# skmhrk1209/VSRD

Hardware: AMD Instinct MI355X
Metric: rendered rays/sec (fwd+bwd) per GPU, KITTI-360 376×1408, 16 instances (higher is better)
Workload: dtype f32

## Files before the change

__graft_entry__.py:

```python
import os
import subprocess
import sys

ROOT = os.path.dirname(os.path.abspath(__file__))
if ROOT not in sys.path:
    sys.path.insert(0, ROOT)

CSRC = os.path.join(ROOT, "vsrd_amd", "csrc")
LIB_DIR = os.path.join(ROOT, "vsrd_amd", "lib")
LIB = os.path.join(LIB_DIR, "libvsrd_hip.so")
HIPCC = os.environ.get("HIPCC", "/opt/rocm/bin/hipcc")
COMMON_FLAGS = ["--offload-arch=gfx950", "-O3", "-std=c++17", "-fPIC", "-ffp-contract=fast"]
if os.environ.get("VSRD_SLP", "0") != "1":
    COMMON_FLAGS.append("-fno-slp-vectorize")
COMMON_FLAGS += os.environ.get("VSRD_HIPCC_EXTRA", "").split()
SCHED_FLAGS = [] if os.environ.get("VSRD_SCHED", "iterative-ilp") == "default" else \
    ["-mllvm", "-amdgpu-sched-strategy=" + os.environ.get("VSRD_SCHED", "iterative-ilp")]
UNITS = [("api.hip", SCHED_FLAGS), ("split_front.hip", [])]
HIPCC_FLAGS = COMMON_FLAGS + SCHED_FLAGS


def _stale(target, sources):
    if not os.path.exists(target):
        return True
    t = os.path.getmtime(target)
    return any(os.path.getmtime(s) > t for s in sources)


def compile_library(output, extra_flags=()):
    staged = f"{output}.{os.getpid()}.tmp.so"
    objects, running = [], []
    try:
        for name, unit_flags in UNITS:
            obj = f"{output}.{os.getpid()}.{name}.o"
            objects.append(obj)
            running.append(subprocess.Popen([HIPCC, *COMMON_FLAGS, *unit_flags, *extra_flags, "-c", os.path.join(CSRC, name), "-o", obj], cwd=ROOT))
        codes = [p.wait() for p in running]
        if any(codes):
            raise subprocess.CalledProcessError(next(c for c in codes if c), "hipcc -c")
        subprocess.run([HIPCC, "--offload-arch=gfx950", "-shared", "-fPIC", "-o", staged, *objects], check=True, cwd=ROOT)
        os.replace(staged, output)
    finally:
        for path in [staged, *objects]:
            if os.path.exists(path):
                os.remove(path)


def build(force=False):
    os.makedirs(LIB_DIR, exist_ok=True)
    sources = [os.path.join(CSRC, f) for f in sorted(os.listdir(CSRC))]
    sources.append(os.path.join(ROOT, "include", "vsrd_hip.h"))
# ... 64 lines not shown
```

include/vsrd_hip.h:

```cpp
#ifndef VSRD_HIP_H
#define VSRD_HIP_H

#include <stddef.h>
#include <stdint.h>

#ifdef __cplusplus
extern "C" {
#endif

#define VSRD_ABI_VERSION 12

#define VSRD_OK 0
#define VSRD_E_INVALID_ARGUMENT (-1)
#define VSRD_E_UNSUPPORTED (-2)
#define VSRD_E_LAUNCH (-3)
#define VSRD_E_WORKSPACE (-4)

#define VSRD_MAX_INSTANCES 64
#define VSRD_MAX_SAMPLES 256
#define VSRD_INSTANCE_STRIDE 16
#define VSRD_MLP_WEIGHTS 1617

#define VSRD_FRAME_HEADER_HAS_VIEWS 0x10000
typedef struct vsrd_frame_header {
// ... 310 lines not shown
} vsrd_frame_log_config;

int32_t vsrd_frame_log(const vsrd_frame_log_config* log, void* stream);

#define VSRD_PATCH_MAX_VIEWS 32
#define VSRD_PATCH_MAX_PIXELS 256
#define VSRD_PATCH_MAX_RAYS 65535
typedef struct vsrd_patch_correlation_config {
    int32_t num_views;
    int32_t num_rays;
    int32_t height, width;
    int32_t patch_width;
    int32_t patch_height;
    int32_t top_k;
    int32_t target_view;
    float sample_epsilon;
    float correlation_epsilon;
} vsrd_patch_correlation_config;

int32_t vsrd_grayscale_images(const float* images, int32_t num_views, int32_t height, int32_t width, float* gray, void* stream);

size_t vsrd_patch_correlation_workspace_bytes(int32_t num_views, int32_t num_rays, int32_t patch_pixels);

int32_t vsrd_patch_correlation_forward(const vsrd_patch_correlation_config* config, const float* gray, const float* intrinsics, const float* extrinsics,
                                       const int32_t* pixels, const float* positions, const float* normals, const uint8_t* converged,
                                       void* workspace, size_t workspace_bytes, float* loss, float* stats,
                                       float* patches, float* coefficients, int32_t* selected, void* stream);

int32_t vsrd_patch_correlation_backward(const vsrd_patch_correlation_config* config, const float* gray, const float* intrinsics, const float* extrinsics,
                                        const int32_t* pixels, const float* positions, const float* normals, const uint8_t* converged,
                                        void* workspace, size_t workspace_bytes, const float* stats, const float* grad_loss,
                                        float* grad_positions, float* grad_normals, void* stream);

#define VSRD_HYPER_LAYERS 5
#define VSRD_HYPER_WIDTH 256
typedef struct vsrd_hypernetwork {
    int32_t num_instances;
    int32_t num_outputs;
    float beta1, beta2, adam_epsilon, lr_gamma;
    vsrd_adam_tensors embeddings;
    vsrd_adam_tensors weight_v[VSRD_HYPER_LAYERS];
    vsrd_adam_tensors weight_g[VSRD_HYPER_LAYERS];
    vsrd_adam_tensors bias[VSRD_HYPER_LAYERS];
    vsrd_adam_tensors norm_weight[VSRD_HYPER_LAYERS - 1];
    vsrd_adam_tensors norm_bias[VSRD_HYPER_LAYERS - 1];
    int32_t num_frames;
    int64_t frame_stride;
} vsrd_hypernetwork;

size_t vsrd_hypernetwork_workspace_bytes(int32_t num_instances);

int32_t vsrd_hypernetwork_forward(const vsrd_hypernetwork* net, void* workspace, size_t workspace_bytes,
                                  float* mlp_weights, float* centred, void* stream);

int32_t vsrd_hypernetwork_backward_step(const vsrd_hypernetwork* net, void* workspace, size_t workspace_bytes,
                                        const float* grad_mlp_weights, float grad_scale, void* stream);

int32_t vsrd_hypernetwork_forward_with_header(const vsrd_hypernetwork* net, void* workspace, size_t workspace_bytes,
                                              float* mlp_weights, float* centred, const vsrd_frame_header* frame_header, void* stream);
int32_t vsrd_hypernetwork_backward_step_with_header(const vsrd_hypernetwork* net, void* workspace, size_t workspace_bytes,
                                                    const float* grad_mlp_weights, float grad_scale, const vsrd_frame_header* frame_header, void* stream);

int32_t vsrd_centre_mlp_weights(const float* mlp_weights, int32_t num_instances, float* centred, void* stream);

int32_t vsrd_selftest_wave(const float* in64, float* out576, void* stream);
int32_t vsrd_selftest_gelu(const float* x, int32_t n, float* out, void* stream);
// ... 6 lines not shown
```

vsrd_amd/csrc/api.hip:

```cpp
#include <cstdio>
#include <cstdlib>
#include "../../include/vsrd_hip.h"
#include "aux_kernels.h"
#include "quad_step.h"
#include "matching.h"
#include "ray_sampling.h"
#include "projection.h"
#include "frame_step.h"
#include "hypernetwork.h"
#include "frame_ingest.h"
#include "frame_labels.h"
#include "frame_group_labels.h"
#include "frame_masks.h"
#include "frame_metrics.h"
#include "frame_log.h"
#include "patch_correlation.h"
#include "launch.h"

namespace {

using namespace vsrd;

constexpr int kMaxBlocks = 16384;

// ... 194 lines not shown
    bool rows;
    bool quad, full;
    int lanes, rays_per_wave, shape_instances;
    int rounds;
    size_t lds_floats;
    size_t num_groups;
    size_t flag_bytes;
};
RowsPlan plan_rows(int num_instances, int num_distances, int num_rays, uint32_t flags, bool allowed) {
    RowsPlan r = {};
    r.rows = allowed && !(flags & VSRD_FLAG_STEP_WAVE_PER_RAY) && num_instances <= kPairMaxInstances && num_distances <= 2 * kPairMaxSamples;
    if (!r.rows) return r;
    const int S = (num_distances + 1) / 2;
    r.quad = num_instances <= kQuadMaxInstances && num_distances <= 2 * kQuadMaxSamples;
    r.lanes = r.quad ? kRowLanes : 32;
    r.rays_per_wave = kWave / r.lanes;
    r.shape_instances = r.quad ? kQuadMaxInstances : kPairMaxInstances;
    r.full = num_distances == 8 * r.lanes && 2 * num_instances > r.shape_instances && !switches().no_full_shape;
    r.rounds = (r.quad && S <= r.lanes) ? 1 : (S <= 2 * r.lanes ? 2 : 4);
    r.lds_floats = static_cast<size_t>(quad_lds_floats(S, r.full ? r.shape_instances : num_instances, r.lanes));
    r.num_groups = (static_cast<size_t>(num_rays) + r.rays_per_wave - 1) / r.rays_per_wave;
    r.flag_bytes = 16 + ((r.num_groups + 15) & ~static_cast<size_t>(15));
    return r;
}

bool cap_to_workspace(size_t bytes, int width, size_t flag_bytes, Geometry* g) {
    const int waves_per_block = g->threads / kWave;
    if (flag_bytes + static_cast<size_t>(waves_per_block) * width * sizeof(float) > bytes) return false;
    const int max_waves = static_cast<int>((bytes - flag_bytes) / sizeof(float) / width);
    if (g->blocks * waves_per_block > max_waves) g->blocks = max_waves / waves_per_block;
    return true;
}

template <typename Kernel, typename... Args>
void launch_hot_then_rest(Kernel hot, Kernel rest, const Geometry& g, hipStream_t s, Args... args) {
    hipLaunchKernelGGL(hot, dim3(g.blocks), dim3(g.threads), g.lds_bytes, s, args...);
    hipLaunchKernelGGL(rest, dim3(g.blocks), dim3(g.threads), g.lds_bytes, s, args...);
}

constexpr size_t kSeedBudgetBytes = size_t(6) << 30;
constexpr int kFrontBlocks = 512;
constexpr int kMlpAdjointBlocks = 4096;
constexpr int kPairBlocks = 1024;

struct ResidualStepPlan {
    int rounds, chunk, front_blocks, front_waves, slots_per_item, items_per_instance;
    bool pair;
    long long slots_per_instance;
    size_t front_lds;
    size_t box_partials, loss_partials, jets, box_extra, counter, segment_sums, seeds, item_rows, masks, item_flags, images, total_bytes;
};

long long size_chunk(ResidualStepPlan* p, long long chunk, int N) {
    p->chunk = static_cast<int>(chunk);
    const long long want = (chunk + kMaxWavesPerBlock - 1) / kMaxWavesPerBlock;
    p->front_blocks = static_cast<int>(want > kFrontBlocks ? kFrontBlocks : want);
    p->front_waves = p->front_blocks * kMaxWavesPerBlock;
    p->slots_per_instance = chunk * p->rounds;
    return (p->slots_per_instance * N) / 16384;
}

void lay_out(ResidualStepPlan* p, int N, long long per_item, size_t loss_floats, bool with_images) {
    p->slots_per_item = static_cast<int>(per_item);
    p->items_per_instance = static_cast<int>((p->slots_per_instance + per_item - 1) / per_item);
    size_t at = 0;
    auto take = [&](size_t floats) { const size_t here = at; at += (floats + 3) & ~size_t(3); return here; };
// ... 375 lines not shown
    if (residual && config->num_rays > 0 && !(config->flags & VSRD_FLAG_RESIDUAL_SINGLE_KERNEL)) {
        bool taken = false;
        const int32_t status = render_backward_split(field, config, origins, directions, distances, num_distances, grad_labels, grad_gradients,
                                                     grad_weights, workspace, workspace_bytes, grad_instances, grad_mlp_weights, stream, &taken);
        if (taken) return status;
    }
    const hipStream_t s = static_cast<hipStream_t>(stream);
    const int row = N * kGradStride;
    const int mlp_row = N * kMlpWeights;
    if (config->num_rays == 0) {
        if (residual && hipMemsetAsync(grad_mlp_weights, 0, mlp_row * sizeof(float), s) != hipSuccess) return VSRD_E_LAUNCH;
        return hipMemsetAsync(grad_instances, 0, row * sizeof(float), s) == hipSuccess ? VSRD_OK : VSRD_E_LAUNCH;
    }
    Geometry g;
    const FieldArgs f = field_args(field);
    RenderArgs c = render_args(config);
    c.sh.inv_t = f.inv_t;
    const RowsPlan r = plan_rows(N, num_distances, config->num_rays, config->flags, !residual && !grad_gradients && !grad_weights);
    if (r.rows) {
        if (!plan(static_cast<int>(r.num_groups), r.lds_floats, &g)) return VSRD_E_UNSUPPORTED;
        if (!cap_to_workspace(workspace_bytes, row, r.flag_bytes, &g)) return VSRD_E_WORKSPACE;
        const int num_waves = g.blocks * (g.threads / kWave);
        float* partials = static_cast<float*>(workspace);
        unsigned char* redo_flags = reinterpret_cast<unsigned char*>(partials + static_cast<size_t>(num_waves) * row);
        if (hipMemsetAsync(redo_flags, 0, 16, s) != hipSuccess) return VSRD_E_LAUNCH;
        for_bool(r.full, [&](auto full) {
            auto launch = [&](auto hot, auto rest) {
                launch_hot_then_rest(hot, rest, g, s, f, field->instances, c, origins, directions, distances, num_distances, grad_labels, partials, redo_flags);
            };
            if (r.quad) launch(render_backward_quad_kernel<true, decltype(full)::value>, render_backward_quad_kernel<false, false>);
            else launch(render_backward_pair_kernel<true, decltype(full)::value>, render_backward_pair_kernel<false, false>);
        });
        if (launch_status() != VSRD_OK) return VSRD_E_LAUNCH;
        hipLaunchKernelGGL(reduce_partials_kernel, dim3(row), dim3(256), 0, s, partials, num_waves, row, grad_instances);
        return launch_status();
    }
    if (!plan(config->num_rays, static_cast<size_t>(backward_lds_floats(num_distances, N, residual)), &g)) return VSRD_E_UNSUPPORTED;
    if (residual && g.threads > kResidualWaves * kWave) return VSRD_E_UNSUPPORTED;
    if (residual && g.blocks > kMaxBlocksResidual) g.blocks = kMaxBlocksResidual;
    const OneKernelWorkspace w = one_kernel_workspace(workspace, N, residual);
    bool known = false;
    for_bool(residual, [&](auto res) {
        known = for_rounds<1, 2, 4>(rounds_for(num_distances - 1), [&](auto k) {
            constexpr auto kernel = render_backward_kernel<decltype(k)::value, decltype(res)::value>;
            fit_to_residency(kernel, &g);
            if (residual && g.blocks > kMaxBlocksResidual) g.blocks = kMaxBlocksResidual;
            hipLaunchKernelGGL(kernel, dim3(g.blocks), dim3(g.threads), g.lds_bytes, s, f, field->instances, field->mlp_weights, c, origins, directions, distances,
                               num_distances, grad_labels, grad_gradients, grad_weights, w.partials, w.mlp_partials, w.jets, w.seeds);
        });
    });
    if (!known) return VSRD_E_UNSUPPORTED;
    if (launch_status() != VSRD_OK) return VSRD_E_LAUNCH;
    const int num_waves = g.blocks * (g.threads / kWave);
    hipLaunchKernelGGL(reduce_partials_kernel, dim3(row), dim3(256), 0, s, w.partials, num_waves, row, grad_instances);
    if (residual)
        hipLaunchKernelGGL(reduce_partials_kernel, dim3(mlp_row), dim3(256), 0, s, w.mlp_partials, num_waves, mlp_row, grad_mlp_weights);
    return launch_status();
}

int32_t vsrd_render_hierarchical_forward(const vsrd_field* field, const vsrd_render_config* config,
                                         const float* origins, const float* directions,
                                         const float* u_coarse, const float* u_fine,
                                         float* labels, float* distances, float* gradients, float* weights, float* coarse_weights,
                                         float* u_coarse_out, float* u_fine_out, void* stream) {
    if (config != nullptr && config->num_frames > 1) return VSRD_E_UNSUPPORTED;
    if (!valid_field(field) || !valid_config(config)) return VSRD_E_INVALID_ARGUMENT;
    if (config->num_rays == 0) return VSRD_OK;
// ... 142 lines not shown
    const int num_waves = g.blocks * (g.threads / kWave);
    float* partials = static_cast<float*>(workspace);
    float* loss_partials = partials + static_cast<size_t>(num_waves) * row;
    unsigned char* redo_flags = reinterpret_cast<unsigned char*>(loss_partials + num_waves);
    int32_t status = VSRD_OK;
    bool known = true;
    if (r.rows) {
        auto launch = [&](auto hot, auto rest) {
            if ((status = opt_in_lds(hot, g.lds_bytes)) != VSRD_OK || (status = opt_in_lds(rest, g.lds_bytes)) != VSRD_OK) return;
            if (hipMemsetAsync(redo_flags, 0, 16, s) != hipSuccess) { status = VSRD_E_LAUNCH; return; }
            launch_hot_then_rest(hot, rest, g, s, f, field->instances, c, origins, directions, u_coarse, u_fine, targets, instance_weights, loss_scale, labels, partials,
                                 loss_partials, redo_flags);
        };
        const bool yaw_only = (config->flags & VSRD_FLAG_YAW_GRADIENTS) != 0u;
        if (r.quad && r.full) for_bool(yaw_only, [&](auto y) {
            launch(render_silhouette_quad_kernel<4, true, true, decltype(y)::value>, render_silhouette_quad_kernel<4, false, false>); });
        else if (r.full) for_bool(yaw_only, [&](auto y) {
            launch(render_silhouette_pair_kernel<4, true, true, decltype(y)::value>, render_silhouette_pair_kernel<4, false, false>); });
        else if (r.quad) known = for_rounds<1, 2, 4>(r.rounds, [&](auto k) {
            launch(render_silhouette_quad_kernel<decltype(k)::value, true, false>, render_silhouette_quad_kernel<decltype(k)::value, false, false>); });
        else known = for_rounds<2, 4>(r.rounds, [&](auto k) {
            launch(render_silhouette_pair_kernel<decltype(k)::value, true, false>, render_silhouette_pair_kernel<decltype(k)::value, false, false>); });
    } else {
        known = for_rounds<1, 2, 4>(rounds, [&](auto k) {
            constexpr auto kernel = render_silhouette_kernel<decltype(k)::value>;
            if ((status = opt_in_lds(kernel, g.lds_bytes)) != VSRD_OK) return;
            hipLaunchKernelGGL(kernel, dim3(g.blocks), dim3(g.threads), g.lds_bytes, s, f, field->instances, c, origins, directions, u_coarse, u_fine, targets,
                               instance_weights, loss_scale, labels, partials, loss_partials);
        });
    }
    if (!known) return VSRD_E_UNSUPPORTED;
    if (status != VSRD_OK) return status;
    if (launch_status() != VSRD_OK) return VSRD_E_LAUNCH;
    hipLaunchKernelGGL(reduce_partials_kernel, dim3(row + 1), dim3(256), 0, s, partials, num_waves, row, grad_instances, nullptr, loss_partials, 1, loss);
    return launch_status();
}

static int32_t residual_step_single_kernel(const vsrd_field* field, const vsrd_render_config* config,
                                  const float* origins, const float* directions, const float* u_coarse, const float* u_fine,
                                  const float* targets, const float* instance_weights, float loss_scale, float eikonal_ratio,
                                  void* workspace, size_t workspace_bytes,
                                  float* losses, float* grad_instances, float* grad_mlp_weights, float* labels, void* stream) {
    if (!valid_field(field) || !valid_config(config, true) || !workspace || !losses || !grad_instances || !grad_mlp_weights) return VSRD_E_INVALID_ARGUMENT;
    if (field->mlp_weights == nullptr) return VSRD_E_INVALID_ARGUMENT;
    const int N = field->num_instances;
    if (workspace_bytes < vsrd_workspace_bytes(N, 1)) return VSRD_E_WORKSPACE;
    const hipStream_t s = static_cast<hipStream_t>(stream);
    const int row = N * kGradStride, mlp_row = N * kMlpWeights;
    if (config->num_rays == 0) {
        if (hipMemsetAsync(losses, 0, 2 * sizeof(float), s) != hipSuccess) return VSRD_E_LAUNCH;
        if (hipMemsetAsync(grad_mlp_weights, 0, mlp_row * sizeof(float), s) != hipSuccess) return VSRD_E_LAUNCH;
        return hipMemsetAsync(grad_instances, 0, row * sizeof(float), s) == hipSuccess ? VSRD_OK : VSRD_E_LAUNCH;
    }
    if (!origins || !directions || !targets) return VSRD_E_INVALID_ARGUMENT;
    const int S = config->num_samples;
    const int num_points = 2 * S - 1;
    const int rounds = rounds_for(num_points);
    Geometry g;
    if (!plan(config->num_rays, static_cast<size_t>(residual_step_lds_floats(S, N)), &g)) return VSRD_E_UNSUPPORTED;
    if (g.threads > kResidualWaves * kWave) return VSRD_E_UNSUPPORTED;
    if (g.blocks > kMaxBlocksResidual) g.blocks = kMaxBlocksResidual;
    const FieldArgs f = field_args(field);
    RenderArgs c = render_args(config);
    c.sh.inv_t = f.inv_t;
    const int num_waves = g.blocks * (g.threads / kWave);
    const OneKernelWorkspace w = one_kernel_workspace(workspace, N, true);
    float* loss_partials = w.partials + static_cast<size_t>(num_waves) * row;
// ... 415 lines not shown

size_t vsrd_patch_correlation_workspace_bytes(int32_t num_views, int32_t num_rays, int32_t patch_pixels) {
    return valid_patch_shape(num_views, num_rays, patch_pixels) ? patch_workspace_floats(num_views, num_rays) * sizeof(float) : 0;
}

int32_t vsrd_patch_correlation_forward(const vsrd_patch_correlation_config* config, const float* gray, const float* intrinsics, const float* extrinsics,
                                       const int32_t* pixels, const float* positions, const float* normals, const uint8_t* converged,
                                       void* workspace, size_t workspace_bytes, float* loss, float* stats,
                                       float* patches, float* coefficients, int32_t* selected, void* stream) {
    PatchArgs a;
    const int32_t status = patch_args(config, gray, intrinsics, extrinsics, pixels, positions, normals, converged, workspace, workspace_bytes, &a);
    if (status != VSRD_OK) return status;
    if (!loss || !stats) return VSRD_E_INVALID_ARGUMENT;
    const hipStream_t s = static_cast<hipStream_t>(stream);
    hipLaunchKernelGGL(patch_constants_kernel, dim3(1), dim3(kWave), 0, s, a);
    hipLaunchKernelGGL(patch_correlation_forward_kernel, dim3(a.num_rays), dim3(kPatchThreads), 0, s, a, patches, coefficients, selected);
    hipLaunchKernelGGL(patch_loss_kernel, dim3(1), dim3(kWave), 0, s, a, loss, stats);
    return launch_status();
}

int32_t vsrd_patch_correlation_backward(const vsrd_patch_correlation_config* config, const float* gray, const float* intrinsics, const float* extrinsics,
                                        const int32_t* pixels, const float* positions, const float* normals, const uint8_t* converged,
                                        void* workspace, size_t workspace_bytes, const float* stats, const float* grad_loss,
                                        float* grad_positions, float* grad_normals, void* stream) {
    PatchArgs a;
    const int32_t status = patch_args(config, gray, intrinsics, extrinsics, pixels, positions, normals, converged, workspace, workspace_bytes, &a);
    if (status != VSRD_OK) return status;
    if (!stats || !grad_loss || !grad_positions || !grad_normals) return VSRD_E_INVALID_ARGUMENT;
    const hipStream_t s = static_cast<hipStream_t>(stream);
    hipLaunchKernelGGL(patch_constants_kernel, dim3(1), dim3(kWave), 0, s, a);
    hipLaunchKernelGGL(patch_correlation_backward_kernel, dim3(a.num_rays), dim3(kPatchThreads), 0, s, a, stats, grad_loss, grad_positions, grad_normals);
    return launch_status();
}

namespace {
struct HyperPlan {
    size_t activations;
    size_t inv_norm;
    size_t gz;
    size_t partials;
    size_t norm_partials;
    size_t total;
    int final_blocks;
};
static HyperPlan plan_hypernetwork(int num_instances) {
    const size_t slab = static_cast<size_t>(num_instances) * kHyperWidth;
    HyperPlan p;
    p.final_blocks = (kMlpWeights + kHyperWaves - 1) / kHyperWaves;
    p.activations = 0;
    p.inv_norm = p.activations + (VSRD_HYPER_LAYERS - 1) * slab;
    p.gz = p.inv_norm + (VSRD_HYPER_LAYERS - 1) * kHyperWidth + kMlpWbarFloats;
    p.partials = p.gz + (VSRD_HYPER_LAYERS) * slab;
    p.norm_partials = p.partials + static_cast<size_t>(p.final_blocks) * slab;
    p.total = p.norm_partials + (VSRD_HYPER_LAYERS - 1) * 2 * slab;
    return p;
}
static bool valid_hypernetwork(const vsrd_hypernetwork* net) {
    if (!net || net->num_instances < 1 || net->num_instances > VSRD_MAX_INSTANCES || net->num_outputs != kMlpWeights) return false;
    if (!valid_adam(net->embeddings)) return false;
    for (int l = 0; l < VSRD_HYPER_LAYERS; ++l) {
        if (!valid_adam(net->weight_v[l]) || !valid_adam(net->weight_g[l]) || !valid_adam(net->bias[l])) return false;
        if (l + 1 < VSRD_HYPER_LAYERS && (!valid_adam(net->norm_weight[l]) || !valid_adam(net->norm_bias[l]))) return false;
    }
    return true;
}
}
// ... 197 lines not shown
```

vsrd_amd/csrc/frame_step.h:

```cpp
#pragma once
#include "matching.h"
#include "projection.h"

namespace vsrd {

constexpr int kFrameThreads = 256;
constexpr int kFrameMaxBoxes = 64;
constexpr int kFrameMaxViews = 32;
constexpr int kBoxEdges = 12;

struct FrameStepArgs {
    int num_boxes, num_views;
    float height, width, epsilon;
    float location_lo[3], location_hi[3], dimension_lo[3], dimension_hi[3];
    int num_steps;
    float max_temperature, min_temperature, max_std, min_std;
    float weight_iou, weight_l1, weight_silhouette;
    float beta1, beta2, adam_epsilon, lr_gamma;
    long long frame_stride;
    const FrameHeader* header;
};

__host__ __device__ constexpr size_t frame_scratch_floats(int num_views, int num_boxes) {
    return static_cast<size_t>(num_views) * num_boxes * (4 + 4 + 4 + 24);
}

__device__ __forceinline__ float lerp_torch(float a, float b, float w) {
    const float diff = b - a;
    return (fabsf(w) < 0.5f) ? (a + w * diff) : (b - diff * (1.0f - w));
}
__device__ __forceinline__ float sigmoid_precise(float x) { return 1.0f / (1.0f + expf(-x)); }

struct DecodedBox {
    float sig_l[3], sig_d[3];
    float loc[3], dim[3];
    float norm, c, s;
};

__device__ __forceinline__ DecodedBox decode_box(const FrameStepArgs& a, const float* raw_loc, const float* raw_dim, const float* raw_ori) {
    DecodedBox b;
#pragma unroll
    for (int j = 0; j < 3; ++j) {
        b.sig_l[j] = sigmoid_precise(raw_loc[j]);
        b.sig_d[j] = sigmoid_precise(raw_dim[j]);
        b.loc[j] = lerp_torch(a.location_lo[j], a.location_hi[j], b.sig_l[j]);
        b.dim[j] = lerp_torch(a.dimension_lo[j], a.dimension_hi[j], b.sig_d[j]);
    }
    b.norm = fmaxf(sqrtf(raw_ori[0] * raw_ori[0] + raw_ori[1] * raw_ori[1]), 1.0e-12f);
    b.c = raw_ori[0] / b.norm;
    b.s = raw_ori[1] / b.norm;
    return b;
}

__device__ __forceinline__ void unit_corner(int k, float* u) {
    const int table[8][3] = {{-1, -1, 1}, {1, -1, 1}, {1, -1, -1}, {-1, -1, -1}, {-1, 1, 1}, {1, 1, 1}, {1, 1, -1}, {-1, 1, -1}};
    u[0] = static_cast<float>(table[k][0]); u[1] = static_cast<float>(table[k][1]); u[2] = static_cast<float>(table[k][2]);
}

__device__ __forceinline__ float dmax_first(float a, float b) { return (a > b) ? 1.0f : ((a == b) ? 0.5f : 0.0f); }
__device__ __forceinline__ float dmin_first(float a, float b) { return (a < b) ? 1.0f : ((a == b) ? 0.5f : 0.0f); }

__device__ __forceinline__ float diou_loss(const float* p, const float* g, float* grad) {
    const float x1 = p[0], y1 = p[1], x2 = p[2], y2 = p[3], x1g = g[0], y1g = g[1], x2g = g[2], y2g = g[3];
    const float eps = 1.0e-7f;
    const float ix1 = fmaxf(x1, x1g), iy1 = fmaxf(y1, y1g), ix2 = fminf(x2, x2g), iy2 = fminf(y2, y2g);
    const bool overlap = (iy2 > iy1) && (ix2 > ix1);
    const float iw = ix2 - ix1, ih = iy2 - iy1;
    const float inter = overlap ? iw * ih : 0.0f;
    const float uni = (x2 - x1) * (y2 - y1) + (x2g - x1g) * (y2g - y1g) - inter;
    const float wx = fmaxf(x2, x2g) - fminf(x1, x1g), wy = fmaxf(y2, y2g) - fminf(y1, y1g);
    const float diagonal = wx * wx + wy * wy + eps;
    const float cxd = (x1 + x2) / 2.0f - (x1g + x2g) / 2.0f, cyd = (y1 + y2) / 2.0f - (y1g + y2g) / 2.0f;
    const float centres = cxd * cxd + cyd * cyd;
    const float ue = uni + eps;
    const float dI[4] = {overlap ? -ih * dmax_first(x1, x1g) : 0.0f, overlap ? -iw * dmax_first(y1, y1g) : 0.0f,
                         overlap ? ih * dmin_first(x2, x2g) : 0.0f, overlap ? iw * dmin_first(y2, y2g) : 0.0f};
    const float dA[4] = {-(y2 - y1), -(x2 - x1), (y2 - y1), (x2 - x1)};
    const float dD[4] = {-2.0f * wx * dmin_first(x1, x1g), -2.0f * wy * dmin_first(y1, y1g), 2.0f * wx * dmax_first(x2, x2g), 2.0f * wy * dmax_first(y2, y2g)};
    const float dC[4] = {cxd, cyd, cxd, cyd};
#pragma unroll
    for (int k = 0; k < 4; ++k) {
        const float dU = dA[k] - dI[k];
        grad[k] = -(dI[k] * ue - inter * dU) / (ue * ue) + (dC[k] * diagonal - centres * dD[k]) / (diagonal * diagonal);
    }
    return 1.0f - inter / ue + centres / diagonal;
}

struct FrameBuffers {
    const float* raw_locations;
// ... 429 lines not shown
```

vsrd_amd/csrc/render_kernels.h:

```cpp
#pragma once
#include "render.h"

namespace vsrd {

constexpr int kMaxWavesPerBlock = 4;
constexpr int kBlockThreads = kMaxWavesPerBlock * kWave;

__device__ __forceinline__ int waves_per_block() { return static_cast<int>(blockDim.x) >> 6; }
constexpr int kGradStride = kInstanceStride;
constexpr int kSeedFloats = 7;
constexpr int kMlpBatch = 8;

__host__ __device__ constexpr int forward_weights_floats(bool residual) { return residual ? kMlpWbarFloats : 0; }

__host__ __device__ constexpr int backward_lds_floats(int num_distances, int num_instances, bool residual) {
    return (forward_weights_floats(residual) + (residual ? kMlpLdsFloats + kMlpBatch * 4 * num_instances : 0) + num_distances + num_instances +
            num_instances * kGradStride + cull_coef_floats(num_instances) + 3) & ~3;
}

__host__ __device__ constexpr int forward_lds_floats(int num_distances, int num_instances, bool residual = false) {
    return (forward_weights_floats(residual) + num_distances + num_instances * kWave + cull_coef_floats(num_instances) + 3) & ~3;
}

__host__ __device__ constexpr int hierarchical_lds_floats(int num_samples, int num_instances, bool residual) {
// ... 1556 lines not shown
        float* dst = box_extra + i * kGradStride + (idx - kMlpWbarFloats);
        *dst = (accumulate ? *dst : 0.0f) + total;
    }
}

__global__ __launch_bounds__(256) void reduce_partials_kernel(const float* __restrict__ partials, int num_waves, int row, float* __restrict__ out,
                                                              const float* __restrict__ extra = nullptr,
                                                              const float* __restrict__ partials2 = nullptr, int row2 = 0, float* __restrict__ out2 = nullptr,
                                                              long long frame_stride = 0, const FrameHeader* __restrict__ frame_header = nullptr) {
    if (frame_stride != 0) {
        const long long shift = frame_shift(frame_stride, blockIdx.y);
        VSRD_OF_FRAME(partials, shift); VSRD_OF_FRAME(out, shift); VSRD_OF_FRAME(extra, shift); VSRD_OF_FRAME(partials2, shift); VSRD_OF_FRAME(out2, shift);
        VSRD_OF_FRAME(frame_header, shift);
    }
    __shared__ float scratch[256 / kWave];
    const bool second = static_cast<int>(blockIdx.x) >= row;
    const int idx = second ? static_cast<int>(blockIdx.x) - row : static_cast<int>(blockIdx.x);
    if (frame_header != nullptr && !second && idx >= frame_count(frame_header, row / kGradStride) * kGradStride) return;
    const float* table = second ? partials2 : partials;
    const int pitch = second ? row2 : row;
    float acc = 0.0f;
    for (int w = threadIdx.x; w < num_waves; w += blockDim.x) acc += table[static_cast<size_t>(w) * pitch + idx];
    acc = wave_sum(acc);
    if (lane_id() == 0) scratch[threadIdx.x >> 6] = acc;
    __syncthreads();
    if (threadIdx.x == 0) {
        float total = 0.0f;
        for (int k = 0; k < 256 / kWave; ++k) total += scratch[k];
        if (second) out2[idx] = total;
        else out[idx] = total + (extra ? extra[idx] : 0.0f);
    }
}

}
```

vsrd_amd/fields.py:

```python
import functools
from dataclasses import dataclass
from typing import Optional

import torch

from . import _lib


class UnsupportedFieldError(TypeError):
    pass


@dataclass
class FieldBlock:
    instances: torch.Tensor
    temperature: float
    mlp_weights: Optional[torch.Tensor]
    label_indices: Optional[torch.Tensor]
    hard: bool = False
    yaw_gradients: bool = False
    capture_key: Optional[tuple] = None

    @property
    def num_instances(self):
        return self.instances.shape[0]


def pack_instances(locations, orientations, dimensions):
    n = locations.shape[0]
    return torch.cat([locations.reshape(n, 3), orientations.reshape(n, 9), dimensions.reshape(n, 3),
                      locations.new_zeros(n, 1)], dim=-1).to(torch.float32).contiguous()



class _Field:

    def __call__(self, positions):
        from .rendering import evaluate_field
        return evaluate_field(self, positions)


class BoxSDF(_Field):

    def __init__(self, dimension):
        self.dimension = dimension


class Rotation(_Field):

    def __init__(self, sdf, rotation_matrix):
        self.sdf, self.rotation_matrix = sdf, rotation_matrix


class Translation(_Field):

    def __init__(self, sdf, translation_vector):
        self.sdf, self.translation_vector = sdf, translation_vector


class ResidualField(_Field):

# ... 206 lines not shown
```

vsrd_amd/models.py:

```python
import math

import torch
import torch.nn as nn
import torch.nn.functional as F

_UNIT_CORNERS = [[-1, -1, 1], [1, -1, 1], [1, -1, -1], [-1, -1, -1], [-1, 1, 1], [1, 1, 1], [1, 1, -1], [-1, 1, -1]]


def yaw_matrix(cos, sin):
    zero, one = torch.zeros_like(cos), torch.ones_like(cos)
    rows = [torch.stack([cos, zero, sin], -1), torch.stack([zero, one, zero], -1), torch.stack([-sin, zero, cos], -1)]
    return torch.stack(rows, -2)


_corner_cache = {}


def _unit_corners(like):
    key = (like.device, like.dtype)
    if key not in _corner_cache:
        _corner_cache[key] = torch.tensor(_UNIT_CORNERS, dtype=like.dtype, device=like.device)
    return _corner_cache[key]


class BoxParameters3D(nn.Module):

    def __init__(self, batch_size, num_instances, num_features=256,
                 location_range=((-50.0, 1.55 - 1.75 / 2.0 - 5.0, 0.0), (50.0, 1.55 - 1.75 / 2.0 + 5.0, 100.0)),
                 dimension_range=((0.75, 0.75, 1.5), (1.0, 1.0, 2.5))):
        super().__init__()
        self.locations = nn.Parameter(torch.zeros(batch_size, num_instances, 3))
        self.dimensions = nn.Parameter(torch.zeros(batch_size, num_instances, 3))
        self.orientations = nn.Parameter(torch.tensor([1.0, 0.0]).repeat(batch_size, num_instances, 1))
        self.embeddings = nn.Parameter(torch.rand(num_features).repeat(batch_size, num_instances, 1))
        self.register_buffer("location_range", torch.as_tensor(location_range, dtype=torch.float32))
        self.register_buffer("dimension_range", torch.as_tensor(dimension_range, dtype=torch.float32))

    def decode_location(self, raw):
        return torch.lerp(self.location_range[0], self.location_range[1], torch.sigmoid(raw))

    def decode_dimension(self, raw):
        return torch.lerp(self.dimension_range[0], self.dimension_range[1], torch.sigmoid(raw))

    def decode_orientation(self, raw):
        heading = F.normalize(raw, dim=-1)
        return yaw_matrix(heading[..., 0], heading[..., 1])

    @staticmethod
    def decode_box_3d(locations, dimensions, orientations):
        corners = _unit_corners(dimensions) * dimensions.unsqueeze(-2)
        return corners @ orientations.transpose(-2, -1) + locations.unsqueeze(-2)

    @staticmethod
    def encode_box_3d(boxes_3d):
        def mean_edge(a, b):
            return (boxes_3d[..., a, :] - boxes_3d[..., b, :]).norm(dim=-1).mean(-1)
        locations = boxes_3d.mean(-2)
        half = torch.stack([mean_edge([1, 2, 6, 5], [0, 3, 7, 4]), mean_edge([4, 5, 6, 7], [0, 1, 2, 3]),
                            mean_edge([1, 0, 4, 5], [2, 3, 7, 6])], -1) / 2.0
        forward = (boxes_3d[..., [1, 0, 4, 5], :] - boxes_3d[..., [2, 3, 7, 6], :]).mean(-2)
        heading = F.normalize(forward[..., [2, 0]], dim=-1)
        return locations, half, yaw_matrix(heading[..., 0], heading[..., 1])

    def forward(self):
        locations = self.decode_location(self.locations)
        dimensions = self.decode_dimension(self.dimensions)
        orientations = self.decode_orientation(self.orientations)
        return dict(boxes_3d=self.decode_box_3d(locations, dimensions, orientations), locations=locations,
                    dimensions=dimensions, orientations=orientations, embeddings=self.embeddings)


class SinusoidalEncoder(nn.Module):
    def __init__(self, num_frequencies):
        super().__init__()
        self.register_buffer("frequencies", 2.0 ** torch.arange(num_frequencies) * math.pi)

    def forward(self, inputs):
        phase = self.frequencies * inputs.unsqueeze(-1)
        return torch.stack([torch.cos(phase), torch.sin(phase)], dim=-1).flatten(-3, -1)


class HyperDistanceField(nn.Module):

    def __init__(self, in_channels, out_channels_list, hyper_in_channels, hyper_out_channels_list):
        super().__init__()
        fan_in = [in_channels, *out_channels_list]
        fan_out = [*out_channels_list, 1]
        self.num_neurons_list = [(i + 1) * o for i, o in zip(fan_in, fan_out)]
        self.in_channels_list, self.out_channels_list = fan_in, fan_out
        widths = [hyper_in_channels, *hyper_out_channels_list]
        blocks = [nn.Sequential(nn.utils.weight_norm(nn.Linear(a, b)), nn.LayerNorm(b), nn.GELU())
                  for a, b in zip(widths[:-1], widths[1:])]
        blocks.append(nn.Sequential(nn.utils.weight_norm(nn.Linear(widths[-1], sum(self.num_neurons_list)))))
        self.hypernetwork = nn.Sequential(*blocks)

    def distance_field(self, weights, positions):
        features = positions
# ... 11 lines not shown
```

Before: 241.6 million.

## Fuse box parameter decode into HIP kernels and split partial-gradient reduction

Adds a native single-block HIP kernel pair that decodes raw box parameters (sigmoid/lerp, yaw matrix, corners) and computes their gradients. It also emits a packed instance block that pack_instances can reuse instead of concatenating. This replaces the many small PyTorch ops and their launches per step. Separately, the backward partial-gradient reduction becomes a two-stage scheme that writes residues into spare workspace, for more parallelism when the number of waves is large. The risks are tensor-identity bookkeeping through a _vsrd_packed attribute, and workspace aliasing with the residue region.

```diff
diff --git a/__graft_entry__.py b/__graft_entry__.py
--- a/__graft_entry__.py
+++ b/__graft_entry__.py
@@ -16,7 +16,7 @@
 COMMON_FLAGS += os.environ.get("VSRD_HIPCC_EXTRA", "").split()
 SCHED_FLAGS = [] if os.environ.get("VSRD_SCHED", "iterative-ilp") == "default" else \
     ["-mllvm", "-amdgpu-sched-strategy=" + os.environ.get("VSRD_SCHED", "iterative-ilp")]
-UNITS = [("api.hip", SCHED_FLAGS), ("split_front.hip", [])]
+UNITS = [("api.hip", SCHED_FLAGS), ("split_front.hip", []), ("box_decode.hip", ["-ffp-contract=fast-honor-pragmas"])]
 HIPCC_FLAGS = COMMON_FLAGS + SCHED_FLAGS
 
 
diff --git a/include/vsrd_hip.h b/include/vsrd_hip.h
--- a/include/vsrd_hip.h
+++ b/include/vsrd_hip.h
@@ -366,6 +366,16 @@
                                         void* workspace, size_t workspace_bytes, const float* stats, const float* grad_loss,
                                         float* grad_positions, float* grad_normals, void* stream);
 
+int32_t vsrd_box_decode_forward(const float* raw_locations, const float* raw_dimensions, const float* raw_orientations,
+                                const float* location_range, const float* dimension_range, int32_t num_instances,
+                                float* instances, float* locations, float* dimensions, float* orientations, float* boxes_3d, void* stream);
+
+int32_t vsrd_box_decode_backward(const float* raw_locations, const float* raw_dimensions, const float* raw_orientations,
+                                 const float* location_range, const float* dimension_range, int32_t num_instances,
+                                 const float* grad_instances, const float* grad_locations, const float* grad_dimensions,
+                                 const float* grad_orientations, const float* grad_boxes_3d,
+                                 float* grad_raw_locations, float* grad_raw_dimensions, float* grad_raw_orientations, void* stream);
+
 #define VSRD_HYPER_LAYERS 5
 #define VSRD_HYPER_WIDTH 256
 typedef struct vsrd_hypernetwork {
diff --git a/vsrd_amd/csrc/api.hip b/vsrd_amd/csrc/api.hip
--- a/vsrd_amd/csrc/api.hip
+++ b/vsrd_amd/csrc/api.hip
@@ -250,6 +250,21 @@
     return true;
 }
 
+void launch_reduce_rows(const float* partials, int num_waves, int row, float* out, const float* partials2, int row2, float* out2, void* workspace,
+                        size_t bytes, hipStream_t s) {
+    const size_t rows_end = (static_cast<size_t>(num_waves) * (row + row2) * sizeof(float) + 16 + 15) & ~static_cast<size_t>(15);
+    const size_t residue_bytes = (static_cast<size_t>(kReduceResidues) * (row + row2) * sizeof(float) + 15) & ~static_cast<size_t>(15);
+    if (rows_end + residue_bytes > bytes) {
+        hipLaunchKernelGGL(reduce_partials_kernel, dim3(row + row2), dim3(256), 0, s, partials, num_waves, row, out, nullptr, partials2, row2, out2);
+        return;
+    }
+    float* residues = reinterpret_cast<float*>(static_cast<char*>(workspace) + ((bytes - residue_bytes) & ~static_cast<size_t>(15)));
+    float* residues2 = residues + static_cast<size_t>(kReduceResidues) * row;
+    hipLaunchKernelGGL(reduce_partials_residues_kernel, dim3(kReduceResidues, (row + 255) / 256 + (row2 > 0 ? 1 : 0)), dim3(256), 0, s, partials, num_waves, row,
+                       partials2, row2, residues, residues2);
+    hipLaunchKernelGGL(reduce_partials_kernel, dim3(row + row2), dim3(256), 0, s, residues, kReduceResidues, row, out, nullptr, row2 > 0 ? residues2 : nullptr, row2, out2);
+}
+
 template <typename Kernel, typename... Args>
 void launch_hot_then_rest(Kernel hot, Kernel rest, const Geometry& g, hipStream_t s, Args... args) {
     hipLaunchKernelGGL(hot, dim3(g.blocks), dim3(g.threads), g.lds_bytes, s, args...);
@@ -691,7 +706,7 @@
             else launch(render_backward_pair_kernel<true, decltype(full)::value>, render_backward_pair_kernel<false, false>);
         });
         if (launch_status() != VSRD_OK) return VSRD_E_LAUNCH;
-        hipLaunchKernelGGL(reduce_partials_kernel, dim3(row), dim3(256), 0, s, partials, num_waves, row, grad_instances);
+        launch_reduce_rows(partials, num_waves, row, grad_instances, nullptr, 0, nullptr, workspace, workspace_bytes, s);
         return launch_status();
     }
     if (!plan(config->num_rays, static_cast<size_t>(backward_lds_floats(num_distances, N, residual)), &g)) return VSRD_E_UNSUPPORTED;
@@ -900,7 +915,7 @@
     if (!known) return VSRD_E_UNSUPPORTED;
     if (status != VSRD_OK) return status;
     if (launch_status() != VSRD_OK) return VSRD_E_LAUNCH;
-    hipLaunchKernelGGL(reduce_partials_kernel, dim3(row + 1), dim3(256), 0, s, partials, num_waves, row, grad_instances, nullptr, loss_partials, 1, loss);
+    launch_reduce_rows(partials, num_waves, row, grad_instances, loss_partials, 1, loss, workspace, vsrd_workspace_bytes(N, 0), s);
     return launch_status();
 }
 
@@ -1382,6 +1397,7 @@
     hipLaunchKernelGGL(patch_correlation_backward_kernel, dim3(a.num_rays), dim3(kPatchThreads), 0, s, a, stats, grad_loss, grad_positions, grad_normals);
     return launch_status();
 }
+
 
 namespace {
 struct HyperPlan {
diff --git a/vsrd_amd/csrc/box_decode.h b/vsrd_amd/csrc/box_decode.h
--- /dev/null
+++ b/vsrd_amd/csrc/box_decode.h
@@ -0,0 +1,17 @@
+#pragma once
+#include <hip/hip_runtime.h>
+
+namespace vsrd {
+
+__device__ __forceinline__ float lerp_torch(float a, float b, float w) {
+    const float diff = b - a;
+    return (fabsf(w) < 0.5f) ? (a + w * diff) : (b - diff * (1.0f - w));
+}
+__device__ __forceinline__ float sigmoid_precise(float x) { return 1.0f / (1.0f + expf(-x)); }
+
+__device__ __forceinline__ void unit_corner(int k, float* u) {
+    const int table[8][3] = {{-1, -1, 1}, {1, -1, 1}, {1, -1, -1}, {-1, -1, -1}, {-1, 1, 1}, {1, 1, 1}, {1, 1, -1}, {-1, 1, -1}};
+    u[0] = static_cast<float>(table[k][0]); u[1] = static_cast<float>(table[k][1]); u[2] = static_cast<float>(table[k][2]);
+}
+
+}
diff --git a/vsrd_amd/csrc/box_decode.hip b/vsrd_amd/csrc/box_decode.hip
--- /dev/null
+++ b/vsrd_amd/csrc/box_decode.hip
@@ -0,0 +1,157 @@
+#include <hip/hip_runtime.h>
+#include "../../include/vsrd_hip.h"
+#include "box_decode.h"
+
+namespace vsrd {
+
+constexpr int kBoxDecodeThreads = 64;
+static_assert(kBoxDecodeThreads >= VSRD_MAX_INSTANCES, "one thread per box");
+
+struct BoxHeading { float norm, denom, c, s; };
+__device__ __forceinline__ BoxHeading box_heading(float x0, float x1) {
+#pragma clang fp contract(off)
+    BoxHeading h;
+    h.norm = sqrtf(x0 * x0 + x1 * x1);
+    h.denom = fmaxf(h.norm, 1.0e-12f);
+    h.c = x0 / h.denom;
+    h.s = x1 / h.denom;
+    return h;
+}
+
+__device__ __forceinline__ void yaw_rows(float c, float s, float* R) {
+    R[0] = c; R[1] = 0.0f; R[2] = s; R[3] = 0.0f; R[4] = 1.0f; R[5] = 0.0f; R[6] = -s; R[7] = 0.0f; R[8] = c;
+}
+
+__global__ __launch_bounds__(kBoxDecodeThreads) void box_decode_forward_kernel(const float* __restrict__ raw_locations, const float* __restrict__ raw_dimensions,
+                                                                               const float* __restrict__ raw_orientations, const float* __restrict__ location_range,
+                                                                               const float* __restrict__ dimension_range, int N, float* __restrict__ block,
+                                                                               float* __restrict__ locations, float* __restrict__ dimensions,
+                                                                               float* __restrict__ orientations, float* __restrict__ boxes_3d) {
+#pragma clang fp contract(off)
+    const int i = threadIdx.x;
+    if (i >= N) return;
+    float loc[3], dim[3], R[9];
+#pragma unroll
+    for (int j = 0; j < 3; ++j) {
+        loc[j] = lerp_torch(location_range[j], location_range[3 + j], sigmoid_precise(raw_locations[3 * i + j]));
+        dim[j] = lerp_torch(dimension_range[j], dimension_range[3 + j], sigmoid_precise(raw_dimensions[3 * i + j]));
+    }
+    const BoxHeading h = box_heading(raw_orientations[2 * i], raw_orientations[2 * i + 1]);
+    yaw_rows(h.c, h.s, R);
+    float* row = block + 16 * i;
+#pragma unroll
+    for (int j = 0; j < 3; ++j) { row[j] = loc[j]; row[12 + j] = dim[j]; locations[3 * i + j] = loc[j]; dimensions[3 * i + j] = dim[j]; }
+#pragma unroll
+    for (int j = 0; j < 9; ++j) { row[3 + j] = R[j]; orientations[9 * i + j] = R[j]; }
+    row[15] = 0.0f;
+#pragma unroll
+    for (int k = 0; k < 8; ++k) {
+        float u[3];
+        unit_corner(k, u);
+        const float corner[3] = {u[0] * dim[0], u[1] * dim[1], u[2] * dim[2]};
+#pragma unroll
+        for (int r = 0; r < 3; ++r) {
+            const float dot = __fmaf_rn(corner[2], R[3 * r + 2], __fmaf_rn(corner[1], R[3 * r + 1], corner[0] * R[3 * r]));
+            boxes_3d[24 * i + 3 * k + r] = dot + loc[r];
+        }
+    }
+}
+
+__global__ __launch_bounds__(kBoxDecodeThreads) void box_decode_backward_kernel(const float* __restrict__ raw_locations, const float* __restrict__ raw_dimensions,
+                                                                                const float* __restrict__ raw_orientations, const float* __restrict__ location_range,
+                                                                                const float* __restrict__ dimension_range, int N, const float* __restrict__ grad_block,
+                                                                                const float* __restrict__ grad_locations, const float* __restrict__ grad_dimensions,
+                                                                                const float* __restrict__ grad_orientations, const float* __restrict__ grad_boxes_3d,
+                                                                                float* __restrict__ grad_raw_locations, float* __restrict__ grad_raw_dimensions,
+                                                                                float* __restrict__ grad_raw_orientations) {
+#pragma clang fp contract(off)
+    const int i = threadIdx.x;
+    if (i >= N) return;
+    float g_loc[3] = {0.0f, 0.0f, 0.0f}, g_dim[3] = {0.0f, 0.0f, 0.0f}, g_R[9] = {0.0f, 0.0f, 0.0f, 0.0f, 0.0f, 0.0f, 0.0f, 0.0f, 0.0f};
+    bool any = false;
+    auto add = [&](float* acc, float g, bool first) { *acc = first ? g : *acc + g; };
+    if (grad_block) {
+        const float* row = grad_block + 16 * i;
+        for (int j = 0; j < 3; ++j) { add(g_loc + j, row[j], !any); add(g_dim + j, row[12 + j], !any); }
+        for (int j = 0; j < 9; ++j) add(g_R + j, row[3 + j], !any);
+        any = true;
+    }
+    bool any_loc = any, any_dim = any, any_R = any;
+    if (grad_locations) { for (int j = 0; j < 3; ++j) add(g_loc + j, grad_locations[3 * i + j], !any_loc); any_loc = true; }
+    if (grad_dimensions) { for (int j = 0; j < 3; ++j) add(g_dim + j, grad_dimensions[3 * i + j], !any_dim); any_dim = true; }
+    if (grad_orientations) { for (int j = 0; j < 9; ++j) add(g_R + j, grad_orientations[9 * i + j], !any_R); any_R = true; }
+    const BoxHeading h = box_heading(raw_orientations[2 * i], raw_orientations[2 * i + 1]);
+    float sig_l[3], sig_d[3];
+#pragma unroll
+    for (int j = 0; j < 3; ++j) { sig_l[j] = sigmoid_precise(raw_locations[3 * i + j]); sig_d[j] = sigmoid_precise(raw_dimensions[3 * i + j]); }
+    if (grad_boxes_3d) {
+        float R[9], dim[3];
+        yaw_rows(h.c, h.s, R);
+        for (int j = 0; j < 3; ++j) dim[j] = lerp_torch(dimension_range[j], dimension_range[3 + j], sig_d[j]);
+        float b_loc[3] = {0.0f, 0.0f, 0.0f}, b_dim[3] = {0.0f, 0.0f, 0.0f}, b_R[9] = {0.0f, 0.0f, 0.0f, 0.0f, 0.0f, 0.0f, 0.0f, 0.0f, 0.0f};
+#pragma unroll
+        for (int k = 0; k < 8; ++k) {
+            float u[3];
+            unit_corner(k, u);
+            const float* g = grad_boxes_3d + 24 * i + 3 * k;
+            const float corner[3] = {u[0] * dim[0], u[1] * dim[1], u[2] * dim[2]};
+#pragma unroll
+            for (int c = 0; c < 3; ++c) {
+                b_loc[c] += g[c];
+                const float g_corner = __fmaf_rn(g[2], R[6 + c], __fmaf_rn(g[1], R[3 + c], g[0] * R[c]));
+                b_dim[c] += u[c] * g_corner;
+#pragma unroll
+                for (int r = 0; r < 3; ++r) b_R[3 * r + c] = __fmaf_rn(g[r], corner[c], b_R[3 * r + c]);
+            }
+        }
+        for (int j = 0; j < 3; ++j) { add(g_loc + j, b_loc[j], !any_loc); add(g_dim + j, b_dim[j], !any_dim); }
+        for (int j = 0; j < 9; ++j) add(g_R + j, b_R[j], !any_R);
+    }
+#pragma unroll
+    for (int j = 0; j < 3; ++j) {
+        const float gl = g_loc[j] * (location_range[3 + j] - location_range[j]);
+        const float gd = g_dim[j] * (dimension_range[3 + j] - dimension_range[j]);
+        grad_raw_locations[3 * i + j] = (gl * (1.0f - sig_l[j])) * sig_l[j];
+        grad_raw_dimensions[3 * i + j] = (gd * (1.0f - sig_d[j])) * sig_d[j];
+    }
+    const float x[2] = {raw_orientations[2 * i], raw_orientations[2 * i + 1]};
+    const float g_h[2] = {g_R[0] + g_R[8], g_R[2] + (-g_R[6])};
+    const float g_denom = (-g_h[0]) * ((x[0] / h.denom) / h.denom) + (-g_h[1]) * ((x[1] / h.denom) / h.denom);
+    const float g_norm = (h.norm >= 1.0e-12f) ? g_denom : 0.0f;
+#pragma unroll
+    for (int j = 0; j < 2; ++j) {
+        const float direction = (h.norm == 0.0f) ? 0.0f : x[j] / h.norm;
+        grad_raw_orientations[2 * i + j] = g_h[j] / h.denom + g_norm * direction;
+    }
+}
+
+}
+
+extern "C" {
+
+int32_t vsrd_box_decode_forward(const float* raw_locations, const float* raw_dimensions, const float* raw_orientations,
+                                const float* location_range, const float* dimension_range, int32_t num_instances,
+                                float* instances, float* locations, float* dimensions, float* orientations, float* boxes_3d, void* stream) {
+    if (num_instances < 1 || num_instances > VSRD_MAX_INSTANCES || !raw_locations || !raw_dimensions || !raw_orientations || !location_range || !dimension_range ||
+        !instances || !locations || !dimensions || !orientations || !boxes_3d)
+        return VSRD_E_INVALID_ARGUMENT;
+    hipLaunchKernelGGL(vsrd::box_decode_forward_kernel, dim3(1), dim3(vsrd::kBoxDecodeThreads), 0, static_cast<hipStream_t>(stream), raw_locations, raw_dimensions,
+                       raw_orientations, location_range, dimension_range, num_instances, instances, locations, dimensions, orientations, boxes_3d);
+    return hipGetLastError() == hipSuccess ? VSRD_OK : VSRD_E_LAUNCH;
+}
+
+int32_t vsrd_box_decode_backward(const float* raw_locations, const float* raw_dimensions, const float* raw_orientations,
+                                 const float* location_range, const float* dimension_range, int32_t num_instances,
+                                 const float* grad_instances, const float* grad_locations, const float* grad_dimensions,
+                                 const float* grad_orientations, const float* grad_boxes_3d,
+                                 float* grad_raw_locations, float* grad_raw_dimensions, float* grad_raw_orientations, void* stream) {
+    if (num_instances < 1 || num_instances > VSRD_MAX_INSTANCES || !raw_locations || !raw_dimensions || !raw_orientations || !location_range || !dimension_range ||
+        !grad_raw_locations || !grad_raw_dimensions || !grad_raw_orientations)
+        return VSRD_E_INVALID_ARGUMENT;
+    hipLaunchKernelGGL(vsrd::box_decode_backward_kernel, dim3(1), dim3(vsrd::kBoxDecodeThreads), 0, static_cast<hipStream_t>(stream), raw_locations, raw_dimensions,
+                       raw_orientations, location_range, dimension_range, num_instances, grad_instances, grad_locations, grad_dimensions, grad_orientations,
+                       grad_boxes_3d, grad_raw_locations, grad_raw_dimensions, grad_raw_orientations);
+    return hipGetLastError() == hipSuccess ? VSRD_OK : VSRD_E_LAUNCH;
+}
+
+}
diff --git a/vsrd_amd/csrc/frame_step.h b/vsrd_amd/csrc/frame_step.h
--- a/vsrd_amd/csrc/frame_step.h
+++ b/vsrd_amd/csrc/frame_step.h
@@ -1,6 +1,7 @@
 #pragma once
 #include "matching.h"
 #include "projection.h"
+#include "box_decode.h"
 
 namespace vsrd {
 
@@ -25,12 +26,6 @@
     return static_cast<size_t>(num_views) * num_boxes * (4 + 4 + 4 + 24);
 }
 
-__device__ __forceinline__ float lerp_torch(float a, float b, float w) {
-    const float diff = b - a;
-    return (fabsf(w) < 0.5f) ? (a + w * diff) : (b - diff * (1.0f - w));
-}
-__device__ __forceinline__ float sigmoid_precise(float x) { return 1.0f / (1.0f + expf(-x)); }
-
 struct DecodedBox {
     float sig_l[3], sig_d[3];
     float loc[3], dim[3];
@@ -50,11 +45,6 @@
     b.c = raw_ori[0] / b.norm;
     b.s = raw_ori[1] / b.norm;
     return b;
-}
-
-__device__ __forceinline__ void unit_corner(int k, float* u) {
-    const int table[8][3] = {{-1, -1, 1}, {1, -1, 1}, {1, -1, -1}, {-1, -1, -1}, {-1, 1, 1}, {1, 1, 1}, {1, 1, -1}, {-1, 1, -1}};
-    u[0] = static_cast<float>(table[k][0]); u[1] = static_cast<float>(table[k][1]); u[2] = static_cast<float>(table[k][2]);
 }
 
 __device__ __forceinline__ float dmax_first(float a, float b) { return (a > b) ? 1.0f : ((a == b) ? 0.5f : 0.0f); }
diff --git a/vsrd_amd/csrc/render_kernels.h b/vsrd_amd/csrc/render_kernels.h
--- a/vsrd_amd/csrc/render_kernels.h
+++ b/vsrd_amd/csrc/render_kernels.h
@@ -1612,4 +1612,29 @@
     }
 }
 
-}
+constexpr int kReduceResidues = 256;
+constexpr int kReduceDepth = 16;
+__global__ __launch_bounds__(256) void reduce_partials_residues_kernel(const float* __restrict__ partials, int num_waves, int row,
+                                                                       const float* __restrict__ partials2, int row2,
+                                                                       float* __restrict__ residues, float* __restrict__ residues2) {
+    const int tiles = (row + 255) >> 8;
+    const bool second = static_cast<int>(blockIdx.y) >= tiles;
+    const float* table = second ? partials2 : partials;
+    const int pitch = second ? row2 : row;
+    const int idx = (second ? 0 : static_cast<int>(blockIdx.y) << 8) + static_cast<int>(threadIdx.x);
+    if (idx >= pitch) return;
+    table += idx;
+    float acc = 0.0f;
+    int w = blockIdx.x;
+    for (; w + (kReduceDepth - 1) * kReduceResidues < num_waves; w += kReduceDepth * kReduceResidues) {
+        float v[kReduceDepth];
+#pragma unroll
+        for (int k = 0; k < kReduceDepth; ++k) v[k] = table[static_cast<size_t>(w + k * kReduceResidues) * pitch];
+#pragma unroll
+        for (int k = 0; k < kReduceDepth; ++k) acc += v[k];
+    }
+    for (; w < num_waves; w += kReduceResidues) acc += table[static_cast<size_t>(w) * pitch];
+    (second ? residues2 : residues)[static_cast<size_t>(blockIdx.x) * pitch + idx] = acc;
+}
+
+}
diff --git a/vsrd_amd/fields.py b/vsrd_amd/fields.py
--- a/vsrd_amd/fields.py
+++ b/vsrd_amd/fields.py
@@ -26,7 +26,24 @@
         return self.instances.shape[0]
 
 
+def _decoded_block(locations, orientations, dimensions):
+    def origin(t):
+        return t._base if t._base is not None else t
+    record = getattr(origin(locations), "_vsrd_packed", None)
+    if record is None:
+        return None
+    block, own_orientations, own_dimensions = record
+    pairs = ((locations, origin(locations)), (orientations, own_orientations), (dimensions, own_dimensions))
+    for given, own in pairs:
+        if origin(given) is not own or given.data_ptr() != own.data_ptr() or given.numel() != own.numel() or not given.is_contiguous() or own._version != 0:
+            return None
+    return block if block._version == 0 else None
+
+
 def pack_instances(locations, orientations, dimensions):
+    block = _decoded_block(locations, orientations, dimensions)
+    if block is not None:
+        return block
     n = locations.shape[0]
     return torch.cat([locations.reshape(n, 3), orientations.reshape(n, 9), dimensions.reshape(n, 3),
                       locations.new_zeros(n, 1)], dim=-1).to(torch.float32).contiguous()
diff --git a/vsrd_amd/models.py b/vsrd_amd/models.py
--- a/vsrd_amd/models.py
+++ b/vsrd_amd/models.py
@@ -3,6 +3,8 @@
 import torch
 import torch.nn as nn
 import torch.nn.functional as F
+
+from . import _lib
 
 _UNIT_CORNERS = [[-1, -1, 1], [1, -1, 1], [1, -1, -1], [-1, -1, -1], [-1, 1, 1], [1, 1, 1], [1, 1, -1], [-1, 1, -1]]
 
@@ -21,6 +23,33 @@
     if key not in _corner_cache:
         _corner_cache[key] = torch.tensor(_UNIT_CORNERS, dtype=like.dtype, device=like.device)
     return _corner_cache[key]
+
+
+class _BoxDecode(torch.autograd.Function):
+
+    @staticmethod
+    def forward(ctx, raw_locations, raw_dimensions, raw_orientations, location_range, dimension_range):
+        lib = _lib.load()
+        n = raw_locations.shape[1]
+        raws = [t.detach().contiguous() for t in (raw_locations, raw_dimensions, raw_orientations, location_range, dimension_range)]
+        new = raws[0].new_empty
+        block, locations, dimensions, orientations, boxes_3d = new(n, 16), new(1, n, 3), new(1, n, 3), new(1, n, 3, 3), new(1, n, 8, 3)
+        _lib.check(lib.vsrd_box_decode_forward(*(_lib.ptr(t) for t in raws), n, _lib.ptr(block), _lib.ptr(locations), _lib.ptr(dimensions),
+                                               _lib.ptr(orientations), _lib.ptr(boxes_3d), _lib.stream()))
+        ctx.save_for_backward(raw_locations, raw_dimensions, raw_orientations, location_range, dimension_range)
+        ctx.set_materialize_grads(False)
+        return block, locations, dimensions, orientations, boxes_3d
+
+    @staticmethod
+    def backward(ctx, *cotangents):
+        lib = _lib.load()
+        raws = [t.detach().contiguous() for t in ctx.saved_tensors]
+        n = raws[0].shape[1]
+        cotangents = [None if g is None else g.to(torch.float32).contiguous() for g in cotangents]
+        grads = [torch.empty_like(t) for t in raws[:3]]
+        _lib.check(lib.vsrd_box_decode_backward(*(_lib.ptr(t) for t in raws), n, *(_lib.ptr(g) for g in cotangents), *(_lib.ptr(g) for g in grads),
+                                                _lib.stream()))
+        return grads[0], grads[1], grads[2], None, None
 
 
 class BoxParameters3D(nn.Module):
@@ -62,7 +91,17 @@
         heading = F.normalize(forward[..., [2, 0]], dim=-1)
         return locations, half, yaw_matrix(heading[..., 0], heading[..., 1])
 
+    def _native(self):
+        tensors = (self.locations, self.dimensions, self.orientations, self.location_range, self.dimension_range)
+        return (self.locations.is_cuda and self.locations.shape[0] == 1 and 1 <= self.locations.shape[1] <= _lib.MAX_INSTANCES
+                and all(t.dtype == torch.float32 and t.device == self.locations.device for t in tensors))
+
     def forward(self):
+        if self._native():
+            block, locations, dimensions, orientations, boxes_3d = _BoxDecode.apply(*(
+                self.locations, self.dimensions, self.orientations, self.location_range, self.dimension_range))
+            locations._vsrd_packed = (block, orientations, dimensions)
+            return dict(boxes_3d=boxes_3d, locations=locations, dimensions=dimensions, orientations=orientations, embeddings=self.embeddings)
         locations = self.decode_location(self.locations)
         dimensions = self.decode_dimension(self.dimensions)
         orientations = self.decode_orientation(self.orientations)
```

Result: faster. 244.9 million (median of 6 runs) (+1.4%).
